# hszhao/semseg

Hardware: NVIDIA H100
Metric: PSPNet50 473x473 training images/sec (higher is better)
Workload: dtype bf16

## Files before the change

### semseg_b200/csrc/conv_igemm.cu

```cuda
#include "host_common.h"
#include "ptx.cuh"

namespace sb {

constexpr int kBlockM = 128;
constexpr int kBlockK = 64;
constexpr int kConvThreads = 384;
constexpr int kConsumerThreads = 256;
constexpr int kATileBytes = kBlockM * kBlockK * 2;
constexpr int kStageOutBytes = kBlockM * 64 * 2;
constexpr int kMiscBytes = 2048;

template <int BLOCK_N>
struct ConvCfg {
  static constexpr int kBTileBytes = BLOCK_N * kBlockK * 2;
  static constexpr int kStageBytes = kATileBytes + kBTileBytes;
  static constexpr int kStages = (BLOCK_N == 256) ? 4 : (BLOCK_N == 128 ? 6 : 8);
  static constexpr int kSmemBytes = kStages * kStageBytes + 2 * kStageOutBytes + kMiscBytes + 1024;
};

struct ConvKParams {
  int N, H, W;
  int Cin, Cout;
  int taps;
  int bh, bw, tiles_h, tiles_w;
  int n_tiles, num_m_tiles;
  int k_chunks;
  int dh[SEMSEG_MAX_TAPS], dw[SEMSEG_MAX_TAPS], wtap[SEMSEG_MAX_TAPS], img_add[SEMSEG_MAX_TAPS];
  int img_mul;
  int epi_mode, relu;
  const float* scale;
  const float* shift;
  const __nv_bfloat16* residual;
  const __nv_bfloat16* residual_lo;
  int res_pitch;
  int nseg;
  int k_slices, kb_per_slice;
  long long slice_stride;
  float* out_f32;
  int out_pitch;
  float* stats_partial;
};

template <int BLOCK_N, bool kSplit>
__global__ void __launch_bounds__(kConvThreads, 1)
conv_igemm_kernel(const __grid_constant__ CUtensorMap tmA, const __grid_constant__ CUtensorMap tmB,
                  const __grid_constant__ CUtensorMap tmC, const __grid_constant__ CUtensorMap tmA_lo,
                  const __grid_constant__ CUtensorMap tmB_lo, const __grid_constant__ CUtensorMap tmC_lo,
                  const ConvKParams p) {
  using Cfg = ConvCfg<BLOCK_N>;
  constexpr int kStages = Cfg::kStages;
  constexpr int kStageBytes = Cfg::kStageBytes;
  constexpr int kAcc = BLOCK_N / 2;
  const int num_items = p.num_m_tiles * p.n_tiles * p.k_slices;
  auto decode_item = [&](int item, int& m_tile, int& n_tile, int& k_slice) {
    k_slice = item % p.k_slices;
    item /= p.k_slices;
    n_tile = item % p.n_tiles;
    m_tile = item / p.n_tiles;
  };

  extern __shared__ __align__(1024) uint8_t smem_raw[];
  uint8_t* smem = reinterpret_cast<uint8_t*>((reinterpret_cast<uintptr_t>(smem_raw) + 1023) & ~uintptr_t(1023));
  uint8_t* stage_base = smem;
  uint8_t* out_stage = smem + kStages * kStageBytes;
  uint8_t* misc = out_stage + 2 * kStageOutBytes;
  static_assert(kStages <= 16, "barrier area sized for <= 16 stages");
  uint64_t* full_bar = reinterpret_cast<uint64_t*>(misc);
  uint64_t* empty_bar = full_bar + 16;

  const int warp = threadIdx.x >> 5;
  const int lane = threadIdx.x & 31;
  const int nseg = kSplit ? p.nseg : 1;
  const int total_kblk = p.taps * p.k_chunks;
  auto slice_range = [&](int k_slice, int& kblk0, int& kblk1) {
    kblk0 = k_slice * p.kb_per_slice;
    kblk1 = min(kblk0 + p.kb_per_slice, total_kblk);
  };
  const uint32_t stage_tx = static_cast<uint32_t>(p.bh * p.bw) * 128u + static_cast<uint32_t>(Cfg::kBTileBytes);

  if (warp == 0 && lane == 0) {
    tma_prefetch_desc(&tmA);
    tma_prefetch_desc(&tmB);
    tma_prefetch_desc(&tmC);
    if (kSplit) {
      tma_prefetch_desc(&tmA_lo);
      tma_prefetch_desc(&tmB_lo);
      tma_prefetch_desc(&tmC_lo);
    }
    for (int i = 0; i < kStages; ++i) {
      mbar_init(&full_bar[i], 1);
      mbar_init(&empty_bar[i], kConsumerThreads);
    }
    fence_barrier_init();
  }
  if (p.stats_partial != nullptr) {
    float* row = p.stats_partial + static_cast<size_t>(blockIdx.x) * 4 * 3 * p.Cout;
    for (int i = threadIdx.x; i < 4 * 3 * p.Cout; i += kConvThreads) row[i] = 0.f;
  }
  __syncthreads();

  if (warp < 4) {
    setmaxnreg_dec<40>();
    if (warp == 0 && elect_one()) {
      int it = 0;
      for (int item = blockIdx.x; item < num_items; item += gridDim.x) {
        int m_tile, n_tile, k_slice, kblk0, kblk1;
        decode_item(item, m_tile, n_tile, k_slice);
        slice_range(k_slice, kblk0, kblk1);
        const int tiles_per_img = p.tiles_h * p.tiles_w;
        const int img = m_tile / tiles_per_img;
        const int rem = m_tile - img * tiles_per_img;
        const int h0 = (rem / p.tiles_w) * p.bh;
        const int w0 = (rem % p.tiles_w) * p.bw;
        const int n0 = n_tile * BLOCK_N;
        for (int kb = kblk0 * nseg; kb < kblk1 * nseg; ++kb, ++it) {
          const int s = it % kStages;
          const uint32_t par = (it / kStages) & 1;
          mbar_wait(&empty_bar[s], par ^ 1);
          const int ks = kb / nseg;
          const int seg = kb - ks * nseg;
          const int cb = ks / p.taps;
          const int t = ks - cb * p.taps;
          const CUtensorMap* mA = (kSplit && seg == 1) ? &tmA_lo : &tmA;
          const CUtensorMap* mB = (kSplit && seg == 2) ? &tmB_lo : &tmB;
          uint8_t* a_dst = stage_base + s * kStageBytes;
          uint8_t* b_dst = a_dst + kATileBytes;
          mbar_expect_tx(&full_bar[s], stage_tx);
          tma_load_4d(a_dst, mA, &full_bar[s], cb * kBlockK, w0 + p.dw[t], h0 + p.dh[t],
                      img * p.img_mul + p.img_add[t]);
          tma_load_3d(b_dst, mB, &full_bar[s], cb * kBlockK, n0, p.wtap[t]);
        }
      }
    }
  } else {
    setmaxnreg_inc<232>();
    const int ct = threadIdx.x - 128;
    const int wg = ct >> 7;
    const int wq = (ct >> 5) & 3;
    const int r_base = wg * 64 + wq * 16 + (lane >> 2);
    const int cq = 2 * (lane & 3);
    int it = 0;
    int store_buf = 0;
    float acc[kAcc];
    for (int item = blockIdx.x; item < num_items; item += gridDim.x) {
      int m_tile, n_tile, k_slice, kblk0, kblk1;
      decode_item(item, m_tile, n_tile, k_slice);
      slice_range(k_slice, kblk0, kblk1);
      const int num_kb = (kblk1 - kblk0) * nseg;
      int prev_s = -1;
#pragma unroll
      for (int i = 0; i < kAcc; ++i) acc[i] = 0.f;
      for (int kb = 0; kb < num_kb; ++kb, ++it) {
        const int s = it % kStages;
        const uint32_t par = (it / kStages) & 1;
        mbar_wait(&full_bar[s], par);
        const uint32_t a_addr = smem_u32(stage_base + s * kStageBytes) + static_cast<uint32_t>(wg * 64 * 128);
        const uint32_t b_addr = smem_u32(stage_base + s * kStageBytes + kATileBytes);
        const uint64_t adesc = make_wgmma_desc_sw128(a_addr, 16, 1024);
        const uint64_t bdesc = make_wgmma_desc_sw128(b_addr, 16, 1024);
        wgmma_fence_operand(acc);
        wgmma_fence();
#pragma unroll
        for (int k = 0; k < kBlockK / 16; ++k)
          wgmma_bf16<BLOCK_N, 0, 0>(acc, adesc + static_cast<uint64_t>(k * 2), bdesc + static_cast<uint64_t>(k * 2),
                                    (kb > 0 || k > 0) ? 1u : 0u);
        wgmma_commit();
        wgmma_wait<1>();
        wgmma_fence_operand(acc);
        if (prev_s >= 0) mbar_arrive(&empty_bar[prev_s]);
        prev_s = s;
      }
      wgmma_wait<0>();
      wgmma_fence_operand(acc);
      if (prev_s >= 0) mbar_arrive(&empty_bar[prev_s]);

      const int tiles_per_img = p.tiles_h * p.tiles_w;
      const int img = m_tile / tiles_per_img;
      const int rem = m_tile - img * tiles_per_img;
      const int h0 = (rem / p.tiles_w) * p.bh;
      const int w0 = (rem % p.tiles_w) * p.bw;
      const int n0 = n_tile * BLOCK_N;
      auto row_ok = [&](int r) {
        const int hi = r / p.bw, wi = r - (r / p.bw) * p.bw;
        return (r < p.bh * p.bw) && (h0 + hi < p.H) && (w0 + wi < p.W);
      };
      auto row_pix = [&](int r) {
        const int hi = r / p.bw, wi = r - hi * p.bw;
        return (static_cast<long long>(img) * p.H + (h0 + hi)) * p.W + (w0 + wi);
      };
      bool rv[2];
      long long pix[2];
#pragma unroll
      for (int i = 0; i < 2; ++i) {
        rv[i] = row_ok(r_base + 8 * i);
        pix[i] = row_pix(r_base + 8 * i);
      }
      constexpr int kChunks = BLOCK_N / 64;
#pragma unroll
      for (int ch = 0; ch < kChunks; ++ch) {
        const int c0 = n0 + ch * 64;
        if (c0 >= p.Cout) break;
        float* a = acc + ch * 32;

        if (p.epi_mode == SEMSEG_EPI_F32) {
          const bool bias = p.shift != nullptr && k_slice == 0;
          const bool pairs = ((p.out_pitch | p.slice_stride) & 1) == 0 &&
                             (reinterpret_cast<uintptr_t>(p.out_f32) & 7) == 0;
#pragma unroll
          for (int i = 0; i < 2; ++i) {
            if (!rv[i]) continue;
            float* orow = p.out_f32 + k_slice * p.slice_stride + pix[i] * p.out_pitch;
#pragma unroll
            for (int j = 0; j < 8; ++j) {
              const int c = c0 + 8 * j + cq;
              float v0 = a[4 * j + 2 * i], v1 = a[4 * j + 2 * i + 1];
              if (pairs && c + 1 < p.Cout) {
                if (bias) {
                  v0 += __ldg(p.shift + c);
                  v1 += __ldg(p.shift + c + 1);
                }
                *reinterpret_cast<float2*>(orow + c) = make_float2(v0, v1);
              } else {
                if (c < p.Cout) orow[c] = bias ? v0 + __ldg(p.shift + c) : v0;
                if (c + 1 < p.Cout) orow[c + 1] = bias ? v1 + __ldg(p.shift + c + 1) : v1;
              }
            }
          }
          continue;
        }

        if (p.epi_mode == SEMSEG_EPI_AFFINE) {
          const bool has_res = p.residual != nullptr;
#pragma unroll
          for (int j = 0; j < 8; ++j) {
            const int c = c0 + 8 * j + cq;
            const float sc0 = p.scale ? __ldg(p.scale + c) : 1.f, sc1 = p.scale ? __ldg(p.scale + c + 1) : 1.f;
            const float sh0 = p.shift ? __ldg(p.shift + c) : 0.f, sh1 = p.shift ? __ldg(p.shift + c + 1) : 0.f;
#pragma unroll
            for (int i = 0; i < 2; ++i) {
              float r0 = 0.f, r1 = 0.f;
              if (has_res && rv[i]) {
                const long long ro = pix[i] * p.res_pitch + c;
                float2 f = __bfloat1622float2(*reinterpret_cast<const __nv_bfloat162*>(p.residual + ro));
                if constexpr (kSplit) {
                  const float2 fl = __bfloat1622float2(*reinterpret_cast<const __nv_bfloat162*>(p.residual_lo + ro));
                  f.x += fl.x;
                  f.y += fl.y;
                }
                r0 = f.x;
                r1 = f.y;
              }
              float v0 = fmaf(a[4 * j + 2 * i], sc0, sh0) + r0;
              float v1 = fmaf(a[4 * j + 2 * i + 1], sc1, sh1) + r1;
              if (p.relu) {
                v0 = fmaxf(v0, 0.f);
                v1 = fmaxf(v1, 0.f);
              }
              a[4 * j + 2 * i] = v0;
              a[4 * j + 2 * i + 1] = v1;
            }
          }
        }

        uint8_t* obuf = out_stage + (kSplit ? 0 : store_buf) * kStageOutBytes;
        if (ct == 0) tma_store_wait_read<(kSplit ? 0 : 1)>();
        named_bar_sync(1, kConsumerThreads);
#pragma unroll
        for (int j = 0; j < 8; ++j) {
#pragma unroll
          for (int i = 0; i < 2; ++i) {
            const int r = r_base + 8 * i;
            const float v0 = a[4 * j + 2 * i], v1 = a[4 * j + 2 * i + 1];
            const uint32_t h = pack_bf16x2(v0, v1);
            const int off = r * 128 + ((j ^ (r & 7)) << 4) + cq * 2;
            *reinterpret_cast<uint32_t*>(obuf + off) = h;
            if constexpr (kSplit) {
              const float2 hf = __bfloat1622float2(*reinterpret_cast<const __nv_bfloat162*>(&h));
              *reinterpret_cast<uint32_t*>(obuf + kStageOutBytes + off) = pack_bf16x2(v0 - hf.x, v1 - hf.y);
            }
          }
        }
        fence_proxy_async_smem();
        named_bar_sync(1, kConsumerThreads);
        if (ct == 0) {
          tma_store_4d(&tmC, obuf, c0, w0, h0, img);
          if (kSplit) tma_store_4d(&tmC_lo, obuf + kStageOutBytes, c0, w0, h0, img);
          tma_store_commit();
        }
        if (p.stats_partial != nullptr && p.epi_mode == SEMSEG_EPI_RAW && wg == (ch & 1)) {
          const int g = wq;
          float* st_dst = p.stats_partial + (static_cast<size_t>(blockIdx.x) * 4 + g) * 3 * p.Cout + c0 + 2 * lane;
          float st_old[6];
          st_old[0] = st_dst[0];
          st_old[1] = st_dst[1];
          st_old[2] = st_dst[p.Cout];
          st_old[3] = st_dst[p.Cout + 1];
          st_old[4] = st_dst[2 * p.Cout];
          st_old[5] = st_dst[2 * p.Cout + 1];
          const uint32_t row_msk = __ballot_sync(0xffffffffu, row_ok(g * 32 + lane));
          float s0 = 0.f, s1 = 0.f, q0 = 0.f, q1 = 0.f;
          const uint8_t* base = obuf + (lane & 3) * 4;
          const int chunk16 = lane >> 2;
          auto add_row = [&](int rr, int sw) {
            float2 f = __bfloat1622float2(
                *reinterpret_cast<const __nv_bfloat162*>(base + rr * 128 + ((chunk16 ^ sw) << 4)));
            if constexpr (kSplit) {
              const float2 fl = __bfloat1622float2(*reinterpret_cast<const __nv_bfloat162*>(
                  base + kStageOutBytes + rr * 128 + ((chunk16 ^ sw) << 4)));
              f.x += fl.x;
              f.y += fl.y;
            }
            s0 += f.x;
            s1 += f.y;
            q0 = fmaf(f.x, f.x, q0);
            q1 = fmaf(f.y, f.y, q1);
          };
          if ((row_msk & (row_msk + 1u)) == 0u) {
            const int nr = __popc(row_msk);
            const int nfull = nr >> 3;
            for (int b8 = 0; b8 < nfull; ++b8) {
              const int rr0 = g * 32 + b8 * 8;
#pragma unroll
              for (int k = 0; k < 8; ++k) add_row(rr0 + k, k);
            }
            for (int r = nfull * 8; r < nr; ++r) add_row(g * 32 + r, r & 7);
          } else {
#pragma unroll
            for (int r = 0; r < 32; ++r)
              if ((row_msk >> r) & 1u) add_row(g * 32 + r, r & 7);
          }
          const float nt = static_cast<float>(__popc(row_msk));
          st_dst[0] = st_old[0] + s0;
          st_dst[1] = st_old[1] + s1;
          st_dst[p.Cout] = st_old[2] + q0;
          st_dst[p.Cout + 1] = st_old[3] + q1;
          st_dst[2 * p.Cout] = st_old[4] + nt;
          st_dst[2 * p.Cout + 1] = st_old[5] + nt;
        }
        store_buf ^= 1;
      }
    }
    if (ct == 0) tma_store_wait_all<0>();
  }
}

static int conv_grid(int num_m_tiles, int n_tiles) {
  const int sms = num_sms();
  const long long tiles = static_cast<long long>(num_m_tiles) * n_tiles;
  return static_cast<int>(tiles < sms ? tiles : sms);
}

struct ConvMaps {
  CUtensorMap a, b, c, a_lo, b_lo, c_lo;
};

template <int BLOCK_N>
static int launch_conv(const ConvMaps& tm, const ConvKParams& kp, bool split, int grid, cudaStream_t stream) {
  using Cfg = ConvCfg<BLOCK_N>;
  static std::atomic<bool> attr_set[64];
  int dev = 0;
  SB_CUDA(cudaGetDevice(&dev));
  if (dev < 0 || dev >= 64 || !attr_set[dev].load(std::memory_order_acquire)) {
    SB_CUDA(cudaFuncSetAttribute(conv_igemm_kernel<BLOCK_N, false>, cudaFuncAttributeMaxDynamicSharedMemorySize,
                                 Cfg::kSmemBytes));
    SB_CUDA(cudaFuncSetAttribute(conv_igemm_kernel<BLOCK_N, true>, cudaFuncAttributeMaxDynamicSharedMemorySize,
                                 Cfg::kSmemBytes));
    if (dev >= 0 && dev < 64) attr_set[dev].store(true, std::memory_order_release);
  }
  if (split)
    conv_igemm_kernel<BLOCK_N, true><<<grid, kConvThreads, Cfg::kSmemBytes, stream>>>(tm.a, tm.b, tm.c, tm.a_lo,
                                                                                      tm.b_lo, tm.c_lo, kp);
  else
    conv_igemm_kernel<BLOCK_N, false><<<grid, kConvThreads, Cfg::kSmemBytes, stream>>>(tm.a, tm.b, tm.c, tm.a_lo,
                                                                                       tm.b_lo, tm.c_lo, kp);
  SB_LAUNCHED();
  return SEMSEG_OK;
}

}

static int conv_block_n(int Cout) {
  if (Cout % 256 == 0 || Cout > 128) return 256;
  return Cout > 64 ? 128 : 64;
}

extern "C" int semseg_conv_k_slices(int Cin, int taps, int max_kblocks) {
  if (Cin <= 0 || taps <= 0 || max_kblocks <= 0) return SEMSEG_E_INVALID;
  const int total = taps * sb::cdiv(Cin, sb::kBlockK);
  const int per = sb::cdiv(total, sb::cdiv(total, max_kblocks));
  return sb::cdiv(total, per);
}

extern "C" int semseg_conv_stats_rows(int N, int H, int W, int Cout) {
  if (N <= 0 || H <= 0 || W <= 0 || Cout <= 0) return SEMSEG_E_INVALID;
  int bh, bw;
  sb::choose_box(H, W, sb::kBlockM, &bh, &bw);
  return 4 * sb::conv_grid(N * sb::cdiv(H, bh) * sb::cdiv(W, bw), sb::cdiv(Cout, conv_block_n(Cout)));
}

extern "C" int semseg_conv_fprop(const semseg_conv_desc* d, void* stream_) {
  using namespace sb;
  cudaStream_t stream = static_cast<cudaStream_t>(stream_);
  SB_CHECK_ARG(d != nullptr, "conv: null descriptor");
  SB_CHECK_ARG(d->N > 0 && d->H > 0 && d->W > 0 && d->Cin > 0 && d->Cout > 0, "conv: bad sizes");
  SB_CHECK_ARG(d->taps >= 1 && d->taps <= SEMSEG_MAX_TAPS, "conv: taps=%d out of range", d->taps);
  SB_CHECK_ARG(d->x && d->w, "conv: null x/w");
  SB_CHECK_ARG(d->x_pitch % 8 == 0 && d->x_pitch >= d->Cin, "conv: x_pitch %d must be a multiple of 8 and >= Cin",
               d->x_pitch);
  SB_CHECK_ARG(d->w_cols % 8 == 0 && d->w_cols >= d->Cin, "conv: w_cols %d must be a multiple of 8 and >= Cin",
               d->w_cols);
  SB_CHECK_ARG(d->epi_mode >= 0 && d->epi_mode <= 2, "conv: bad epi_mode");

  ConvKParams kp;
  memset(&kp, 0, sizeof(kp));
  kp.N = d->N; kp.H = d->H; kp.W = d->W; kp.Cin = d->Cin; kp.Cout = d->Cout; kp.taps = d->taps;
  choose_box(d->H, d->W, kBlockM, &kp.bh, &kp.bw);
  kp.tiles_h = cdiv(d->H, kp.bh);
  kp.tiles_w = cdiv(d->W, kp.bw);
  kp.num_m_tiles = d->N * kp.tiles_h * kp.tiles_w;
  kp.k_chunks = cdiv(d->Cin, kBlockK);
  for (int t = 0; t < d->taps; ++t) {
    kp.dh[t] = d->dh[t]; kp.dw[t] = d->dw[t]; kp.wtap[t] = d->wtap[t]; kp.img_add[t] = d->img_add[t];
    SB_CHECK_ARG(d->wtap[t] >= 0 && d->wtap[t] < d->n_wtaps, "conv: wtap[%d]=%d out of range", t, d->wtap[t]);
  }
  kp.img_mul = d->img_mul;
  kp.epi_mode = d->epi_mode; kp.relu = d->relu;
  kp.scale = d->scale; kp.shift = d->shift;
  kp.residual = static_cast<const __nv_bfloat16*>(d->residual); kp.res_pitch = d->res_pitch;
  kp.residual_lo = static_cast<const __nv_bfloat16*>(d->residual_lo);
  const bool split = d->x_lo != nullptr;
  kp.nseg = split ? 3 : 1;
  if (split) {
    SB_CHECK_ARG(d->w_split != 0, "conv: split activations need split weights (w_split)");
    SB_CHECK_ARG(d->epi_mode == SEMSEG_EPI_F32 || d->y_lo != nullptr, "conv: split input needs a split output (y_lo)");
    SB_CHECK_ARG(!d->residual || d->residual_lo, "conv: split input needs a split residual (residual_lo)");
  } else {
    SB_CHECK_ARG(!d->y_lo && !d->residual_lo, "conv: lo planes given without x_lo");
  }
  kp.out_f32 = d->out_f32; kp.out_pitch = d->out_pitch;
  kp.stats_partial = d->stats_partial;

  const int block_n = conv_block_n(d->Cout);
  kp.n_tiles = cdiv(d->Cout, block_n);
  kp.k_slices = 1;
  kp.kb_per_slice = kp.taps * kp.k_chunks;
  kp.slice_stride = 0;
  if (d->k_slices > 1) {
    SB_CHECK_ARG(d->epi_mode == SEMSEG_EPI_F32, "conv: K slicing needs the F32 epilogue (partials are fp32)");
    SB_CHECK_ARG(d->slice_stride >= static_cast<long long>(d->N) * d->H * d->W * d->out_pitch,
                 "conv: slice_stride too small for an [N,H,W,out_pitch] partial");
    kp.kb_per_slice = cdiv(kp.taps * kp.k_chunks, d->k_slices);
    kp.k_slices = cdiv(kp.taps * kp.k_chunks, kp.kb_per_slice);
    SB_CHECK_ARG(kp.k_slices == d->k_slices, "conv: k_slices %d not realisable for %d K blocks (use %d)", d->k_slices,
                 kp.taps * kp.k_chunks, kp.k_slices);
    kp.slice_stride = d->slice_stride;
  }
  const int grid = conv_grid(kp.num_m_tiles, kp.n_tiles * kp.k_slices);

  ConvMaps tm;
  {
    uint64_t dims[4] = {(uint64_t)d->Cin, (uint64_t)d->Win, (uint64_t)d->Hin, (uint64_t)d->Nin};
    uint64_t str[3] = {(uint64_t)d->x_pitch * 2, (uint64_t)d->x_pitch * 2 * d->Win,
                       (uint64_t)d->x_pitch * 2 * d->Win * d->Hin};
    uint32_t box[4] = {(uint32_t)kBlockK, (uint32_t)kp.bw, (uint32_t)kp.bh, 1};
    int r = encode_tmap_bf16(&tm.a, d->x, 4, dims, str, box);
    if (r) return r;
    tm.a_lo = tm.a;
    if (split && (r = encode_tmap_bf16(&tm.a_lo, d->x_lo, 4, dims, str, box))) return r;
  }
  {
    uint64_t dims[3] = {(uint64_t)d->w_cols, (uint64_t)d->w_rows, (uint64_t)d->n_wtaps};
    uint64_t str[2] = {(uint64_t)d->w_cols * 2, (uint64_t)d->w_cols * 2 * d->w_rows};
    uint32_t box[3] = {(uint32_t)kBlockK, (uint32_t)block_n, 1};
    int r = encode_tmap_bf16(&tm.b, d->w, 3, dims, str, box);
    if (r) return r;
    tm.b_lo = tm.b;
    if (split) {
      const __nv_bfloat16* w_lo =
          static_cast<const __nv_bfloat16*>(d->w) + static_cast<size_t>(d->n_wtaps) * d->w_rows * d->w_cols;
      if ((r = encode_tmap_bf16(&tm.b_lo, w_lo, 3, dims, str, box))) return r;
    }
  }
  if (d->epi_mode == SEMSEG_EPI_F32) {
    SB_CHECK_ARG(d->out_f32 != nullptr && d->out_pitch >= d->Cout, "conv: F32 epilogue needs out_f32/out_pitch");
    tm.c = tm.a;
    tm.c_lo = tm.a;
  } else {
    SB_CHECK_ARG(d->y != nullptr, "conv: null y");
    SB_CHECK_ARG(d->Cout % 64 == 0, "conv: bf16 epilogue needs Cout %% 64 == 0 (got %d)", d->Cout);
    SB_CHECK_ARG(d->y_pitch % 8 == 0 && d->y_pitch >= d->Cout, "conv: bad y_pitch %d", d->y_pitch);
    if (d->residual)
      SB_CHECK_ARG(d->res_pitch % 8 == 0 && (reinterpret_cast<uintptr_t>(d->residual) & 3) == 0 &&
                       (reinterpret_cast<uintptr_t>(d->residual_lo) & 3) == 0,
                   "conv: res_pitch must be a multiple of 8 and the residual 4-byte aligned");
    uint64_t dims[4] = {(uint64_t)d->Cout, (uint64_t)d->W, (uint64_t)d->H, (uint64_t)d->N};
    uint64_t str[3] = {(uint64_t)d->y_pitch * 2, (uint64_t)d->y_pitch * 2 * d->W,
                       (uint64_t)d->y_pitch * 2 * d->W * d->H};
    uint32_t box[4] = {64u, (uint32_t)kp.bw, (uint32_t)kp.bh, 1};
    int r = encode_tmap_bf16(&tm.c, d->y, 4, dims, str, box);
    if (r) return r;
    tm.c_lo = tm.c;
    if (split && (r = encode_tmap_bf16(&tm.c_lo, d->y_lo, 4, dims, str, box))) return r;
  }
  switch (block_n) {
    case 256: return launch_conv<256>(tm, kp, split, grid, stream);
    case 128: return launch_conv<128>(tm, kp, split, grid, stream);
    default: return launch_conv<64>(tm, kp, split, grid, stream);
  }
}
```

### semseg_b200/csrc/ptx.cuh

```cuda
#pragma once
#include <cuda.h>
#include <cuda_runtime.h>
#include <cuda_bf16.h>
#include <stdint.h>

namespace sb {

__device__ __forceinline__ uint32_t smem_u32(const void* p) {
  return static_cast<uint32_t>(__cvta_generic_to_shared(p));
}

__device__ __forceinline__ bool elect_one() {
  uint32_t pred = 0;
  asm volatile(
      "{\n"
      ".reg .pred P1;\n"
      "elect.sync _|P1, 0xffffffff;\n"
      "selp.u32 %0, 1, 0, P1;\n"
      "}\n"
      : "=r"(pred));
  return pred != 0;
}

__device__ __forceinline__ void mbar_init(uint64_t* bar, uint32_t count) {
  asm volatile("mbarrier.init.shared::cta.b64 [%0], %1;" ::"r"(smem_u32(bar)), "r"(count));
}
__device__ __forceinline__ void fence_barrier_init() {
  asm volatile("fence.mbarrier_init.release.cluster;" ::: "memory");
}
__device__ __forceinline__ void mbar_expect_tx(uint64_t* bar, uint32_t bytes) {
  asm volatile("mbarrier.arrive.expect_tx.shared::cta.b64 _, [%0], %1;" ::"r"(smem_u32(bar)), "r"(bytes)
               : "memory");
}
__device__ __forceinline__ void mbar_arrive(uint64_t* bar) {
  asm volatile("mbarrier.arrive.shared::cta.b64 _, [%0];" ::"r"(smem_u32(bar)) : "memory");
}
__device__ __forceinline__ bool mbar_try_wait(uint64_t* bar, uint32_t parity) {
  uint32_t ok;
  asm volatile(
      "{\n"
      ".reg .pred P1;\n"
      "mbarrier.try_wait.parity.shared::cta.b64 P1, [%1], %2;\n"
      "selp.u32 %0, 1, 0, P1;\n"
      "}\n"
      : "=r"(ok)
      : "r"(smem_u32(bar)), "r"(parity)
      : "memory");
  return ok != 0;
}
__device__ __forceinline__ void mbar_wait(uint64_t* bar, uint32_t parity) {
  if (mbar_try_wait(bar, parity)) return;
  long long t0 = clock64();
  while (!mbar_try_wait(bar, parity)) {
    if (clock64() - t0 > 8000000000LL) __trap();
  }
}

__device__ __forceinline__ void fence_proxy_async_smem() {
  asm volatile("fence.proxy.async.shared::cta;" ::: "memory");
}
__device__ __forceinline__ void named_bar_sync(uint32_t id, uint32_t nthreads) {
  asm volatile("bar.sync %0, %1;" ::"r"(id), "r"(nthreads) : "memory");
}

__device__ __forceinline__ void tma_prefetch_desc(const CUtensorMap* m) {
  asm volatile("prefetch.tensormap [%0];" ::"l"(reinterpret_cast<uint64_t>(m)) : "memory");
}
__device__ __forceinline__ void tma_load_2d(void* dst, const CUtensorMap* m, uint64_t* bar, int c0, int c1) {
  asm volatile(
      "cp.async.bulk.tensor.2d.shared::cluster.global.mbarrier::complete_tx::bytes [%0], [%1, {%3, %4}], [%2];"
      ::"r"(smem_u32(dst)), "l"(reinterpret_cast<uint64_t>(m)), "r"(smem_u32(bar)), "r"(c0), "r"(c1)
      : "memory");
}
__device__ __forceinline__ void tma_load_3d(void* dst, const CUtensorMap* m, uint64_t* bar, int c0, int c1, int c2) {
  asm volatile(
      "cp.async.bulk.tensor.3d.shared::cluster.global.mbarrier::complete_tx::bytes [%0], [%1, {%3, %4, %5}], [%2];"
      ::"r"(smem_u32(dst)), "l"(reinterpret_cast<uint64_t>(m)), "r"(smem_u32(bar)), "r"(c0), "r"(c1), "r"(c2)
      : "memory");
}
__device__ __forceinline__ void tma_load_4d(void* dst, const CUtensorMap* m, uint64_t* bar, int c0, int c1, int c2,
                                            int c3) {
  asm volatile(
      "cp.async.bulk.tensor.4d.shared::cluster.global.mbarrier::complete_tx::bytes [%0], [%1, {%3, %4, %5, %6}], "
      "[%2];" ::"r"(smem_u32(dst)),
      "l"(reinterpret_cast<uint64_t>(m)), "r"(smem_u32(bar)), "r"(c0), "r"(c1), "r"(c2), "r"(c3)
      : "memory");
}
__device__ __forceinline__ void tma_store_4d(const CUtensorMap* m, const void* src, int c0, int c1, int c2, int c3) {
  asm volatile("cp.async.bulk.tensor.4d.global.shared::cta.bulk_group [%0, {%2, %3, %4, %5}], [%1];" ::"l"(
                   reinterpret_cast<uint64_t>(m)),
               "r"(smem_u32(src)), "r"(c0), "r"(c1), "r"(c2), "r"(c3)
               : "memory");
}
__device__ __forceinline__ void tma_store_commit() { asm volatile("cp.async.bulk.commit_group;" ::: "memory"); }
template <int N>
__device__ __forceinline__ void tma_store_wait_read() {
  asm volatile("cp.async.bulk.wait_group.read %0;" ::"n"(N) : "memory");
}
template <int N>
__device__ __forceinline__ void tma_store_wait_all() {
  asm volatile("cp.async.bulk.wait_group %0;" ::"n"(N) : "memory");
}

template <int R>
__device__ __forceinline__ void setmaxnreg_dec() {
  asm volatile("setmaxnreg.dec.sync.aligned.u32 %0;" ::"n"(R));
}
template <int R>
__device__ __forceinline__ void setmaxnreg_inc() {
  asm volatile("setmaxnreg.inc.sync.aligned.u32 %0;" ::"n"(R));
}

__device__ __forceinline__ void wgmma_fence() { asm volatile("wgmma.fence.sync.aligned;" ::: "memory"); }
__device__ __forceinline__ void wgmma_commit() { asm volatile("wgmma.commit_group.sync.aligned;" ::: "memory"); }
template <int N>
__device__ __forceinline__ void wgmma_wait() {
  asm volatile("wgmma.wait_group.sync.aligned %0;" ::"n"(N) : "memory");
}
template <int R>
__device__ __forceinline__ void wgmma_fence_operand(float (&d)[R]) {
#pragma unroll
  for (int i = 0; i < R; ++i) asm volatile("" : "+f"(d[i])::"memory");
}

__device__ __forceinline__ uint64_t make_wgmma_desc_sw128(uint32_t smem_addr, uint32_t lbo_bytes, uint32_t sbo_bytes) {
  uint64_t d = 0;
  d |= static_cast<uint64_t>((smem_addr & 0x3FFFF) >> 4);
  d |= static_cast<uint64_t>((lbo_bytes >> 4) & 0x3FFF) << 16;
  d |= static_cast<uint64_t>((sbo_bytes >> 4) & 0x3FFF) << 32;
  d |= static_cast<uint64_t>(1) << 62;
  return d;
}

template <int TA, int TB>
__device__ __forceinline__ void wgmma_m64n64(float (&d)[32], uint64_t adesc, uint64_t bdesc, uint32_t accumulate) {
  asm volatile(
      "{\n"
      ".reg .pred p;\n"
      "setp.ne.b32 p, %34, 0;\n"
      "wgmma.mma_async.sync.aligned.m64n64k16.f32.bf16.bf16 "
      "{%0, %1, %2, %3, %4, %5, %6, %7, %8, %9, %10, %11, %12, %13, %14, %15, %16, %17, %18, %19, %20, %21, %22, %23, %24, %25, %26, %27, %28, %29, %30, %31}, "
      "%32, %33, p, 1, 1, %35, %36;\n"
      "}\n"
      : "+f"(d[0]), "+f"(d[1]), "+f"(d[2]), "+f"(d[3]), "+f"(d[4]), "+f"(d[5]), "+f"(d[6]), "+f"(d[7]), "+f"(d[8]), "+f"(d[9]), "+f"(d[10]), "+f"(d[11]), "+f"(d[12]), "+f"(d[13]), "+f"(d[14]), "+f"(d[15]), "+f"(d[16]), "+f"(d[17]), "+f"(d[18]), "+f"(d[19]), "+f"(d[20]), "+f"(d[21]), "+f"(d[22]), "+f"(d[23]), "+f"(d[24]), "+f"(d[25]), "+f"(d[26]), "+f"(d[27]), "+f"(d[28]), "+f"(d[29]), "+f"(d[30]), "+f"(d[31])
      : "l"(adesc), "l"(bdesc), "r"(accumulate), "n"(TA), "n"(TB));
}

template <int TA, int TB>
__device__ __forceinline__ void wgmma_m64n128(float (&d)[64], uint64_t adesc, uint64_t bdesc, uint32_t accumulate) {
  asm volatile(
      "{\n"
      ".reg .pred p;\n"
      "setp.ne.b32 p, %66, 0;\n"
      "wgmma.mma_async.sync.aligned.m64n128k16.f32.bf16.bf16 "
      "{%0, %1, %2, %3, %4, %5, %6, %7, %8, %9, %10, %11, %12, %13, %14, %15, %16, %17, %18, %19, %20, %21, %22, %23, %24, %25, %26, %27, %28, %29, %30, %31, %32, %33, %34, %35, %36, %37, %38, %39, %40, %41, %42, %43, %44, %45, %46, %47, %48, %49, %50, %51, %52, %53, %54, %55, %56, %57, %58, %59, %60, %61, %62, %63}, "
      "%64, %65, p, 1, 1, %67, %68;\n"
      "}\n"
      : "+f"(d[0]), "+f"(d[1]), "+f"(d[2]), "+f"(d[3]), "+f"(d[4]), "+f"(d[5]), "+f"(d[6]), "+f"(d[7]), "+f"(d[8]), "+f"(d[9]), "+f"(d[10]), "+f"(d[11]), "+f"(d[12]), "+f"(d[13]), "+f"(d[14]), "+f"(d[15]), "+f"(d[16]), "+f"(d[17]), "+f"(d[18]), "+f"(d[19]), "+f"(d[20]), "+f"(d[21]), "+f"(d[22]), "+f"(d[23]), "+f"(d[24]), "+f"(d[25]), "+f"(d[26]), "+f"(d[27]), "+f"(d[28]), "+f"(d[29]), "+f"(d[30]), "+f"(d[31]), "+f"(d[32]), "+f"(d[33]), "+f"(d[34]), "+f"(d[35]), "+f"(d[36]), "+f"(d[37]), "+f"(d[38]), "+f"(d[39]), "+f"(d[40]), "+f"(d[41]), "+f"(d[42]), "+f"(d[43]), "+f"(d[44]), "+f"(d[45]), "+f"(d[46]), "+f"(d[47]), "+f"(d[48]), "+f"(d[49]), "+f"(d[50]), "+f"(d[51]), "+f"(d[52]), "+f"(d[53]), "+f"(d[54]), "+f"(d[55]), "+f"(d[56]), "+f"(d[57]), "+f"(d[58]), "+f"(d[59]), "+f"(d[60]), "+f"(d[61]), "+f"(d[62]), "+f"(d[63])
      : "l"(adesc), "l"(bdesc), "r"(accumulate), "n"(TA), "n"(TB));
}

template <int TA, int TB>
__device__ __forceinline__ void wgmma_m64n256(float (&d)[128], uint64_t adesc, uint64_t bdesc, uint32_t accumulate) {
  asm volatile(
      "{\n"
      ".reg .pred p;\n"
      "setp.ne.b32 p, %130, 0;\n"
      "wgmma.mma_async.sync.aligned.m64n256k16.f32.bf16.bf16 "
      "{%0, %1, %2, %3, %4, %5, %6, %7, %8, %9, %10, %11, %12, %13, %14, %15, %16, %17, %18, %19, %20, %21, %22, %23, %24, %25, %26, %27, %28, %29, %30, %31, %32, %33, %34, %35, %36, %37, %38, %39, %40, %41, %42, %43, %44, %45, %46, %47, %48, %49, %50, %51, %52, %53, %54, %55, %56, %57, %58, %59, %60, %61, %62, %63, %64, %65, %66, %67, %68, %69, %70, %71, %72, %73, %74, %75, %76, %77, %78, %79, %80, %81, %82, %83, %84, %85, %86, %87, %88, %89, %90, %91, %92, %93, %94, %95, %96, %97, %98, %99, %100, %101, %102, %103, %104, %105, %106, %107, %108, %109, %110, %111, %112, %113, %114, %115, %116, %117, %118, %119, %120, %121, %122, %123, %124, %125, %126, %127}, "
      "%128, %129, p, 1, 1, %131, %132;\n"
      "}\n"
      : "+f"(d[0]), "+f"(d[1]), "+f"(d[2]), "+f"(d[3]), "+f"(d[4]), "+f"(d[5]), "+f"(d[6]), "+f"(d[7]), "+f"(d[8]), "+f"(d[9]), "+f"(d[10]), "+f"(d[11]), "+f"(d[12]), "+f"(d[13]), "+f"(d[14]), "+f"(d[15]), "+f"(d[16]), "+f"(d[17]), "+f"(d[18]), "+f"(d[19]), "+f"(d[20]), "+f"(d[21]), "+f"(d[22]), "+f"(d[23]), "+f"(d[24]), "+f"(d[25]), "+f"(d[26]), "+f"(d[27]), "+f"(d[28]), "+f"(d[29]), "+f"(d[30]), "+f"(d[31]), "+f"(d[32]), "+f"(d[33]), "+f"(d[34]), "+f"(d[35]), "+f"(d[36]), "+f"(d[37]), "+f"(d[38]), "+f"(d[39]), "+f"(d[40]), "+f"(d[41]), "+f"(d[42]), "+f"(d[43]), "+f"(d[44]), "+f"(d[45]), "+f"(d[46]), "+f"(d[47]), "+f"(d[48]), "+f"(d[49]), "+f"(d[50]), "+f"(d[51]), "+f"(d[52]), "+f"(d[53]), "+f"(d[54]), "+f"(d[55]), "+f"(d[56]), "+f"(d[57]), "+f"(d[58]), "+f"(d[59]), "+f"(d[60]), "+f"(d[61]), "+f"(d[62]), "+f"(d[63]), "+f"(d[64]), "+f"(d[65]), "+f"(d[66]), "+f"(d[67]), "+f"(d[68]), "+f"(d[69]), "+f"(d[70]), "+f"(d[71]), "+f"(d[72]), "+f"(d[73]), "+f"(d[74]), "+f"(d[75]), "+f"(d[76]), "+f"(d[77]), "+f"(d[78]), "+f"(d[79]), "+f"(d[80]), "+f"(d[81]), "+f"(d[82]), "+f"(d[83]), "+f"(d[84]), "+f"(d[85]), "+f"(d[86]), "+f"(d[87]), "+f"(d[88]), "+f"(d[89]), "+f"(d[90]), "+f"(d[91]), "+f"(d[92]), "+f"(d[93]), "+f"(d[94]), "+f"(d[95]), "+f"(d[96]), "+f"(d[97]), "+f"(d[98]), "+f"(d[99]), "+f"(d[100]), "+f"(d[101]), "+f"(d[102]), "+f"(d[103]), "+f"(d[104]), "+f"(d[105]), "+f"(d[106]), "+f"(d[107]), "+f"(d[108]), "+f"(d[109]), "+f"(d[110]), "+f"(d[111]), "+f"(d[112]), "+f"(d[113]), "+f"(d[114]), "+f"(d[115]), "+f"(d[116]), "+f"(d[117]), "+f"(d[118]), "+f"(d[119]), "+f"(d[120]), "+f"(d[121]), "+f"(d[122]), "+f"(d[123]), "+f"(d[124]), "+f"(d[125]), "+f"(d[126]), "+f"(d[127])
      : "l"(adesc), "l"(bdesc), "r"(accumulate), "n"(TA), "n"(TB));
}

template <int N, int TA, int TB>
__device__ __forceinline__ void wgmma_bf16(float (&d)[N / 2], uint64_t adesc, uint64_t bdesc, uint32_t accumulate) {
  static_assert(N == 64 || N == 128 || N == 256, "wgmma N tile");
  if constexpr (N == 64) wgmma_m64n64<TA, TB>(d, adesc, bdesc, accumulate);
  else if constexpr (N == 128) wgmma_m64n128<TA, TB>(d, adesc, bdesc, accumulate);
  else wgmma_m64n256<TA, TB>(d, adesc, bdesc, accumulate);
}

__device__ __forceinline__ uint32_t pack_bf16x2(float lo, float hi) {
  __nv_bfloat162 v = __floats2bfloat162_rn(lo, hi);
  return *reinterpret_cast<uint32_t*>(&v);
}

}
```

Before: 287.2.

## Split conv wave-quantization tail into a second launch with narrower N tiles

When the number of output tiles is not a multiple of the SM count, the persistent conv kernel's last partial wave leaves many SMs idle. The tiles are now split into a main set of full waves and a tail, and the tail runs in a second launch with BLOCK_N divided by 2 or 4. This spreads the tail across more CTAs, using a re-encoded weight tensor map. Stats partial rows are mapped back onto the main grid's CTA rows. The cost is an extra kernel launch and smaller, less efficient tiles in the tail.

```diff
diff --git a/semseg_b200/csrc/conv_igemm.cu b/semseg_b200/csrc/conv_igemm.cu
--- a/semseg_b200/csrc/conv_igemm.cu
+++ b/semseg_b200/csrc/conv_igemm.cu
@@ -40,9 +40,10 @@
   float* out_f32;
   int out_pitch;
   float* stats_partial;
+  int tail_base, tail_items, tail_sub, tail_n_tiles, stats_grid;
 };
 
-template <int BLOCK_N, bool kSplit>
+template <int BLOCK_N, bool kSplit, bool kTail = false>
 __global__ void __launch_bounds__(kConvThreads, 1)
 conv_igemm_kernel(const __grid_constant__ CUtensorMap tmA, const __grid_constant__ CUtensorMap tmB,
                   const __grid_constant__ CUtensorMap tmC, const __grid_constant__ CUtensorMap tmA_lo,
@@ -52,8 +53,15 @@
   constexpr int kStages = Cfg::kStages;
   constexpr int kStageBytes = Cfg::kStageBytes;
   constexpr int kAcc = BLOCK_N / 2;
-  const int num_items = p.num_m_tiles * p.n_tiles * p.k_slices;
+  const int num_items = kTail ? p.tail_items : p.num_m_tiles * p.n_tiles * p.k_slices;
   auto decode_item = [&](int item, int& m_tile, int& n_tile, int& k_slice) {
+    if constexpr (kTail) {
+      const int tile = p.tail_base + item / p.tail_sub;
+      m_tile = tile / p.tail_n_tiles;
+      n_tile = (tile % p.tail_n_tiles) * p.tail_sub + item % p.tail_sub;
+      k_slice = 0;
+      return;
+    }
     k_slice = item % p.k_slices;
     item /= p.k_slices;
     n_tile = item % p.n_tiles;
@@ -94,7 +102,7 @@
     }
     fence_barrier_init();
   }
-  if (p.stats_partial != nullptr) {
+  if (!kTail && p.stats_partial != nullptr) {
     float* row = p.stats_partial + static_cast<size_t>(blockIdx.x) * 4 * 3 * p.Cout;
     for (int i = threadIdx.x; i < 4 * 3 * p.Cout; i += kConvThreads) row[i] = 0.f;
   }
@@ -290,7 +298,9 @@
         }
         if (p.stats_partial != nullptr && p.epi_mode == SEMSEG_EPI_RAW && wg == (ch & 1)) {
           const int g = wq;
-          float* st_dst = p.stats_partial + (static_cast<size_t>(blockIdx.x) * 4 + g) * 3 * p.Cout + c0 + 2 * lane;
+          const uint32_t row_cta =
+              kTail ? static_cast<uint32_t>((p.tail_base + item / p.tail_sub) % p.stats_grid) : blockIdx.x;
+          float* st_dst = p.stats_partial + (static_cast<size_t>(row_cta) * 4 + g) * 3 * p.Cout + c0 + 2 * lane;
           float st_old[6];
           st_old[0] = st_dst[0];
           st_old[1] = st_dst[1];
@@ -355,6 +365,38 @@
   CUtensorMap a, b, c, a_lo, b_lo, c_lo;
 };
 
+static int conv_tail_sub(long long tiles, int n_tiles, int grid, int block_n, long long* main_items) {
+  if (tiles <= grid || tiles % grid == 0) return 0;
+  const long long main = (tiles - tiles % grid) / n_tiles * n_tiles;
+  const long long tail = tiles - main;
+  if (main <= 0 || tail > grid) return 0;
+  int sub = 0;
+  for (int s = 4; s >= 2 && sub == 0; s /= 2)
+    if (block_n / s >= 64 && tail * s <= grid) sub = s;
+  if (sub == 0) return 0;
+  const char* env = getenv("SEMSEG_CONV_TAIL");
+  if (env != nullptr && env[0] == '0' && env[1] == '\0') return 0;
+  *main_items = main;
+  return sub;
+}
+
+template <int BLOCK_N>
+static int launch_conv_tail(const ConvMaps& tm, const ConvKParams& kp, int grid, cudaStream_t stream) {
+  using Cfg = ConvCfg<BLOCK_N>;
+  static std::atomic<bool> attr_set[64];
+  int dev = 0;
+  SB_CUDA(cudaGetDevice(&dev));
+  if (dev < 0 || dev >= 64 || !attr_set[dev].load(std::memory_order_acquire)) {
+    SB_CUDA(cudaFuncSetAttribute(conv_igemm_kernel<BLOCK_N, false, true>, cudaFuncAttributeMaxDynamicSharedMemorySize,
+                                 Cfg::kSmemBytes));
+    if (dev >= 0 && dev < 64) attr_set[dev].store(true, std::memory_order_release);
+  }
+  conv_igemm_kernel<BLOCK_N, false, true><<<grid, kConvThreads, Cfg::kSmemBytes, stream>>>(tm.a, tm.b, tm.c, tm.a_lo,
+                                                                                          tm.b_lo, tm.c_lo, kp);
+  SB_LAUNCHED();
+  return SEMSEG_OK;
+}
+
 template <int BLOCK_N>
 static int launch_conv(const ConvMaps& tm, const ConvKParams& kp, bool split, int grid, cudaStream_t stream) {
   using Cfg = ConvCfg<BLOCK_N>;
@@ -503,9 +545,35 @@
     tm.c_lo = tm.c;
     if (split && (r = encode_tmap_bf16(&tm.c_lo, d->y_lo, 4, dims, str, box))) return r;
   }
-  switch (block_n) {
-    case 256: return launch_conv<256>(tm, kp, split, grid, stream);
-    case 128: return launch_conv<128>(tm, kp, split, grid, stream);
-    default: return launch_conv<64>(tm, kp, split, grid, stream);
-  }
-}
+  long long main_items = 0;
+  const int sub = (split || kp.k_slices > 1 || d->Cout % block_n != 0)
+                      ? 0
+                      : conv_tail_sub(static_cast<long long>(kp.num_m_tiles) * kp.n_tiles, kp.n_tiles, grid, block_n,
+                                      &main_items);
+  ConvKParams kp_tail = kp;
+  if (sub > 0) {
+    kp_tail.tail_base = static_cast<int>(main_items);
+    kp_tail.tail_items = static_cast<int>(static_cast<long long>(kp.num_m_tiles) * kp.n_tiles - main_items) * sub;
+    kp_tail.tail_sub = sub;
+    kp_tail.tail_n_tiles = kp.n_tiles;
+    kp_tail.stats_grid = grid;
+    kp.num_m_tiles = static_cast<int>(main_items / kp.n_tiles);
+  }
+  int r = SEMSEG_OK;
+  if (kp.num_m_tiles > 0) {
+    switch (block_n) {
+      case 256: r = launch_conv<256>(tm, kp, split, grid, stream); break;
+      case 128: r = launch_conv<128>(tm, kp, split, grid, stream); break;
+      default: r = launch_conv<64>(tm, kp, split, grid, stream); break;
+    }
+  }
+  if (r != SEMSEG_OK || sub == 0) return r;
+  {
+    uint64_t dims[3] = {(uint64_t)d->w_cols, (uint64_t)d->w_rows, (uint64_t)d->n_wtaps};
+    uint64_t str[2] = {(uint64_t)d->w_cols * 2, (uint64_t)d->w_cols * 2 * d->w_rows};
+    uint32_t box[3] = {(uint32_t)kBlockK, (uint32_t)(block_n / sub), 1};
+    if ((r = encode_tmap_bf16(&tm.b, d->w, 3, dims, str, box))) return r;
+  }
+  return block_n / sub == 128 ? launch_conv_tail<128>(tm, kp_tail, kp_tail.tail_items, stream)
+                              : launch_conv_tail<64>(tm, kp_tail, kp_tail.tail_items, stream);
+}
```

Result: no change. 287.9 (median of 6 runs) (+0.3%).

## Accumulate BN stats in registers across tiles and prefetch residual into L2

Applied to the files above, without the earlier changes.

Per-tile batch-norm statistics are now gathered in registers by all consumer warps, one column per lane. They are written to the global partial buffer only when the persistent block moves to a different n-tile, which removes a global read-modify-write on every chunk. Residual rows for the affine epilogue are prefetched into L2 before the main loop, so the epilogue load latency overlaps the MMA work. The smem alignment computation also changes to use the shared address. The costs are extra registers and both warpgroups now doing stats work.

```diff
diff --git a/semseg_b200/csrc/conv_igemm.cu b/semseg_b200/csrc/conv_igemm.cu
--- a/semseg_b200/csrc/conv_igemm.cu
+++ b/semseg_b200/csrc/conv_igemm.cu
@@ -60,8 +60,16 @@
     m_tile = item / p.n_tiles;
   };
 
+  auto tile_origin = [&](int m_tile, int& img, int& h0, int& w0) {
+    const int tiles_per_img = p.tiles_h * p.tiles_w;
+    img = m_tile / tiles_per_img;
+    const int rem = m_tile - img * tiles_per_img;
+    h0 = (rem / p.tiles_w) * p.bh;
+    w0 = (rem % p.tiles_w) * p.bw;
+  };
+
   extern __shared__ __align__(1024) uint8_t smem_raw[];
-  uint8_t* smem = reinterpret_cast<uint8_t*>((reinterpret_cast<uintptr_t>(smem_raw) + 1023) & ~uintptr_t(1023));
+  uint8_t* smem = smem_raw + ((1024u - (smem_u32(smem_raw) & 1023u)) & 1023u);
   uint8_t* stage_base = smem;
   uint8_t* out_stage = smem + kStages * kStageBytes;
   uint8_t* misc = out_stage + 2 * kStageOutBytes;
@@ -143,11 +151,30 @@
     int it = 0;
     int store_buf = 0;
     float acc[kAcc];
+    constexpr int kChunks = BLOCK_N / 64;
+    const bool stats = p.stats_partial != nullptr && p.epi_mode == SEMSEG_EPI_RAW;
+    float st_acc[kChunks][2], st_n = 0.f;
+#pragma unroll
+    for (int ch = 0; ch < kChunks; ++ch) st_acc[ch][0] = st_acc[ch][1] = 0.f;
     for (int item = blockIdx.x; item < num_items; item += gridDim.x) {
       int m_tile, n_tile, k_slice, kblk0, kblk1;
       decode_item(item, m_tile, n_tile, k_slice);
       slice_range(k_slice, kblk0, kblk1);
       const int num_kb = (kblk1 - kblk0) * nseg;
+      if (p.epi_mode == SEMSEG_EPI_AFFINE && p.residual != nullptr && (lane & 3) < kChunks) {
+        const int c = n_tile * BLOCK_N + 64 * (lane & 3);
+        int img, h0, w0;
+        tile_origin(m_tile, img, h0, w0);
+#pragma unroll
+        for (int i = 0; i < 2; ++i) {
+          const int r = r_base + 8 * i, hi = r / p.bw, wi = r - hi * p.bw;
+          if (c < p.Cout && r < p.bh * p.bw && h0 + hi < p.H && w0 + wi < p.W) {
+            const long long ro = ((static_cast<long long>(img) * p.H + (h0 + hi)) * p.W + (w0 + wi)) * p.res_pitch + c;
+            prefetch_l2(p.residual + ro);
+            if (kSplit) prefetch_l2(p.residual_lo + ro);
+          }
+        }
+      }
       int prev_s = -1;
 #pragma unroll
       for (int i = 0; i < kAcc; ++i) acc[i] = 0.f;
@@ -175,11 +202,8 @@
       wgmma_fence_operand(acc);
       if (prev_s >= 0) mbar_arrive(&empty_bar[prev_s]);
 
-      const int tiles_per_img = p.tiles_h * p.tiles_w;
-      const int img = m_tile / tiles_per_img;
-      const int rem = m_tile - img * tiles_per_img;
-      const int h0 = (rem / p.tiles_w) * p.bh;
-      const int w0 = (rem % p.tiles_w) * p.bw;
+      int img, h0, w0;
+      tile_origin(m_tile, img, h0, w0);
       const int n0 = n_tile * BLOCK_N;
       auto row_ok = [&](int r) {
         const int hi = r / p.bw, wi = r - (r / p.bw) * p.bw;
@@ -196,7 +220,6 @@
         rv[i] = row_ok(r_base + 8 * i);
         pix[i] = row_pix(r_base + 8 * i);
       }
-      constexpr int kChunks = BLOCK_N / 64;
 #pragma unroll
       for (int ch = 0; ch < kChunks; ++ch) {
         const int c0 = n0 + ch * 64;
@@ -288,57 +311,47 @@
           if (kSplit) tma_store_4d(&tmC_lo, obuf + kStageOutBytes, c0, w0, h0, img);
           tma_store_commit();
         }
-        if (p.stats_partial != nullptr && p.epi_mode == SEMSEG_EPI_RAW && wg == (ch & 1)) {
+        if (stats) {
           const int g = wq;
-          float* st_dst = p.stats_partial + (static_cast<size_t>(blockIdx.x) * 4 + g) * 3 * p.Cout + c0 + 2 * lane;
-          float st_old[6];
-          st_old[0] = st_dst[0];
-          st_old[1] = st_dst[1];
-          st_old[2] = st_dst[p.Cout];
-          st_old[3] = st_dst[p.Cout + 1];
-          st_old[4] = st_dst[2 * p.Cout];
-          st_old[5] = st_dst[2 * p.Cout + 1];
           const uint32_t row_msk = __ballot_sync(0xffffffffu, row_ok(g * 32 + lane));
-          float s0 = 0.f, s1 = 0.f, q0 = 0.f, q1 = 0.f;
-          const uint8_t* base = obuf + (lane & 3) * 4;
-          const int chunk16 = lane >> 2;
-          auto add_row = [&](int rr, int sw) {
-            float2 f = __bfloat1622float2(
-                *reinterpret_cast<const __nv_bfloat162*>(base + rr * 128 + ((chunk16 ^ sw) << 4)));
-            if constexpr (kSplit) {
-              const float2 fl = __bfloat1622float2(*reinterpret_cast<const __nv_bfloat162*>(
-                  base + kStageOutBytes + rr * 128 + ((chunk16 ^ sw) << 4)));
-              f.x += fl.x;
-              f.y += fl.y;
-            }
-            s0 += f.x;
-            s1 += f.y;
-            q0 = fmaf(f.x, f.x, q0);
-            q1 = fmaf(f.y, f.y, q1);
-          };
-          if ((row_msk & (row_msk + 1u)) == 0u) {
-            const int nr = __popc(row_msk);
-            const int nfull = nr >> 3;
-            for (int b8 = 0; b8 < nfull; ++b8) {
-              const int rr0 = g * 32 + b8 * 8;
-#pragma unroll
-              for (int k = 0; k < 8; ++k) add_row(rr0 + k, k);
-            }
-            for (int r = nfull * 8; r < nr; ++r) add_row(g * 32 + r, r & 7);
-          } else {
-#pragma unroll
-            for (int r = 0; r < 32; ++r)
-              if ((row_msk >> r) & 1u) add_row(g * 32 + r, r & 7);
+          float sm = 0.f, sq = 0.f;
+          const int col = 32 * wg + lane;
+          const uint8_t* base = obuf + g * 32 * 128 + (col & 7) * 2;
+          const int chunk16 = col >> 3;
+#pragma unroll
+          for (int r = 0; r < 32; ++r) {
+            const uint8_t* src = base + r * 128 + ((chunk16 ^ (r & 7)) << 4);
+            float f = __bfloat162float(*reinterpret_cast<const __nv_bfloat16*>(src));
+            if constexpr (kSplit) f += __bfloat162float(*reinterpret_cast<const __nv_bfloat16*>(src + kStageOutBytes));
+            f = ((row_msk >> r) & 1u) ? f : 0.f;
+            sm += f;
+            sq = fmaf(f, f, sq);
           }
-          const float nt = static_cast<float>(__popc(row_msk));
-          st_dst[0] = st_old[0] + s0;
-          st_dst[1] = st_old[1] + s1;
-          st_dst[p.Cout] = st_old[2] + q0;
-          st_dst[p.Cout + 1] = st_old[3] + q1;
-          st_dst[2 * p.Cout] = st_old[4] + nt;
-          st_dst[2 * p.Cout + 1] = st_old[5] + nt;
+          st_acc[ch][0] += sm;
+          st_acc[ch][1] += sq;
+          if (ch == 0) st_n += static_cast<float>(__popc(row_msk));
         }
         store_buf ^= 1;
+      }
+      const int next = item + gridDim.x;
+      if (stats && (next >= num_items || (next / p.k_slices) % p.n_tiles != n_tile)) {
+        float* st_dst = p.stats_partial + (static_cast<size_t>(blockIdx.x) * 4 + wq) * 3 * p.Cout + n0 + 32 * wg + lane;
+        float old[kChunks][3];
+#pragma unroll
+        for (int ch = 0; ch < kChunks; ++ch)
+          if (n0 + ch * 64 < p.Cout)
+#pragma unroll
+            for (int v = 0; v < 3; ++v) old[ch][v] = st_dst[ch * 64 + v * p.Cout];
+#pragma unroll
+        for (int ch = 0; ch < kChunks; ++ch) {
+          if (n0 + ch * 64 < p.Cout) {
+            st_dst[ch * 64] = old[ch][0] + st_acc[ch][0];
+            st_dst[ch * 64 + p.Cout] = old[ch][1] + st_acc[ch][1];
+            st_dst[ch * 64 + 2 * p.Cout] = old[ch][2] + st_n;
+          }
+          st_acc[ch][0] = st_acc[ch][1] = 0.f;
+        }
+        st_n = 0.f;
       }
     }
     if (ct == 0) tma_store_wait_all<0>();
diff --git a/semseg_b200/csrc/ptx.cuh b/semseg_b200/csrc/ptx.cuh
--- a/semseg_b200/csrc/ptx.cuh
+++ b/semseg_b200/csrc/ptx.cuh
@@ -61,6 +61,10 @@
 }
 __device__ __forceinline__ void named_bar_sync(uint32_t id, uint32_t nthreads) {
   asm volatile("bar.sync %0, %1;" ::"r"(id), "r"(nthreads) : "memory");
+}
+
+__device__ __forceinline__ void prefetch_l2(const void* ptr) {
+  asm volatile("prefetch.global.L2 [%0];" ::"l"(ptr));
 }
 
 __device__ __forceinline__ void tma_prefetch_desc(const CUtensorMap* m) {
```

Result: faster. 287.4 before, 300.3 after, median of 6 (+4.5%).
